# ittiam-systems/libxaac

Measured on AMD Instinct MI355X. Metric: decoded audio frames/s (1024-spl IMDCT + complex QMF + HQ SBR + parametric stereo, HE-AACv2), higher is better.
Workload: dtype int32

## Files before the change

libxaac_amd/csrc/sbr_core.h:

```cpp
#ifndef XAAC_SBR_CORE_H
#define XAAC_SBR_CORE_H

#include "fx.h"
#include "../../include/xaac_sbr.h"

#ifndef XS_TABLES_DECLARED
#define XS_TABLES_DECLARED
#if defined(__HIPCC__)
#define XAAC_TAB_QUAL static __device__ const
#include "tables_sbr.inc"
#undef XAAC_TAB_QUAL
#else
#include "tables_sbr.inc"
#endif
#endif

#define XS_MAXF XAAC_SBR_MAX_FREQ_COEFFS

FX_HD int32_t xs_shl(int32_t v, int s) { return (int32_t)((uint32_t)v << (s & 31)); }
FX_HD int32_t xs_sar(int32_t v, int s) { return v >> (s & 31); }
FX_HD int xs_pnorm32(int32_t a) { return fx_norm32(a); }
FX_HD int16_t xs_mult16_shl_sat(int16_t a, int16_t b) { return fx_sat16(((int32_t)a * b) >> 15); }
FX_HD int16_t xs_mult16_shl(int16_t a, int16_t b) { return (int16_t)(((int32_t)a * b) >> 15); }
FX_HD int16_t xs_mult16(int16_t a, int16_t b) { return (int16_t)(((int32_t)a * b) >> 16); }
// ... 1815 lines not shown
    st->harm_index = (int16_t)((harm0 + n) & 3);
  }
  cx.sync();
}


FX_HD uint64_t xs_alias_groups_pk(const XsCx &cx, const XsPass &ps, const XsLv &deg1p, const XsLv &alias_red, int nsb,
                                  XsLv &end) {
  XsLv f;
  f.fill(0);
  XS_LANES(l, 0, 64) {
    const int q = l / XS_PK, k = l & (XS_PK - 1);
    if (q < ps.n && k < nsb) f.own(l) = xs_alias_run_bits(k, nsb, deg1p.own(l), alias_red.own(l));
  }
  const uint64_t in_run = xs_ballot(cx, f, 1, 64), red = xs_ballot(cx, f, 2, 64);
  XsLv st;
  st.fill(0);
  XS_LANES(l, 0, 64) st.own(l) = xs_alias_group_at(in_run, red, l, l & ~(XS_PK - 1), nsb, end.own(l)) ? 1 : 0;
  return xs_ballot(cx, st, 1, 64);
}
FX_HD void xs_alias_reduction_pk(const XsCx &cx, const XsPass &ps, XsEnv &v, const XsLv &degp, const XsLv &deg1p, XsWork *w,
                                 uint64_t starts, const XsLv &end, int nsb) {
  if (starts == 0) return;
  XS_LANES(l, 0, 64) {
    w->fold_a[l][0] = v.est.own(l);
    w->fold_a[l][1] = v.gain.own(l);
  }
  cx.sync();
  XS_LANES(s, 0, 64) {
    if (!((starts >> s) & 1)) continue;
    int16_t amp_m, amp_e, gg_m, gg_e;
    xs_avggain(w->fold_a, s, end.own(s), &amp_m, &amp_e, &gg_m, &gg_e, 1);
    w->res_a[s][0] = amp_m;
    w->res_a[s][1] = amp_e;
    w->res_a[s][2] = gg_m;
    w->res_a[s][3] = gg_e;
    w->res_b[s][0] = (int16_t)end.own(s);
  }
  cx.sync();
  XsLv mine;
  mine.fill(-1);
  XS_LANES(l, 0, 64) {
    const int q = l / XS_PK, k = l & (XS_PK - 1);
    if (!(q < ps.n && k < nsb)) continue;
    const uint64_t below = starts & xs_mask_upto(l);
    if (!below) continue;
    const int s = 63 - xs_clz64(below);
    if (l >= w->res_b[s][0]) continue;
    mine.own(l) = s;
    xs_alias_mix_band((int16_t)degp.own(l), (int16_t)deg1p.own(l), k < nsb - 1, w->res_a[s][2], w->res_a[s][3],
                      v.est.own(l), v.gain.own(l), w->fold_b[l]);
  }
  cx.sync();
  XS_LANES(s, 0, 64) {
    if (!((starts >> s) & 1)) continue;
    xs_alias_compensation(w->fold_b, s, end.own(s), w->res_a[s][0], w->res_a[s][1], w->res_b[s][1], w->res_a[s][3]);
  }
  cx.sync();
  XS_LANES(l, 0, 64) {
    const int s = mine.own(l);
    if (s < 0) continue;
    v.gain.own(l) = xs_alias_compensate_band(v.gain.own(l), w->res_b[s][1], w->res_a[s][3]);
  }
  cx.sync();
}
FX_HD bool xs_pack_frame_ok(const XsCx &cx, const xaac_sbr_header *h) {
  const int nhi = cx.uni(h->num_sf_bands[1]), nlo = cx.uni(h->num_sf_bands[0]), nlf = cx.uni(h->num_lf_bands);
  const int sb_start = cx.uni(h->sub_band_start), sb_end = cx.uni(h->sub_band_end), nsb = sb_end - sb_start;
  if (!cx.uni(h->interpol_freq) || nhi < 1 || nlo < 1 || nsb < 1 || nsb > XS_PK) return false;
  if (cx.uni(h->freq_band_tbl_hi[0]) != sb_start || cx.uni(h->freq_band_tbl_lo[0]) != sb_start) return false;
  if (cx.uni(h->freq_band_tbl_hi[nhi]) != sb_end || cx.uni(h->freq_band_tbl_lo[nlo]) != sb_end) return false;
  int32_t bad = 0;
  XS_LANES(c, 0, nlf + 1) bad |= h->freq_band_tbl_lim[c] > nsb;
  return cx.wave_or(bad) == 0;
}

struct XsApplyHq {
  int32_t sl_even, sl_odd;
  int ls, rs, keep, col, step, kk, harm_lane;
  int16_t sg, snz;
  bool tone, noise, fi, live;
  int32_t hr, hr_keep;
};
template <int N, class Q>
FX_HD void xs_apply_slots_hq(const Q &x, XsApplyHq &a, int l, int &ph, int &harm) {
  int32_t rp[N], xr[N], xi[N];
  XS_UNROLL
  for (int j = 0; j < N; j++) rp[j] = XS_TAB_RAND(((ph + j * a.step) & 511) + 1 + a.kk);
  XS_UNROLL
  for (int j = 0; j < N; j++) {
    xr[j] = x(l + j, a.col);
    xi[j] = x.im(l + j, a.col);
  }
  XS_UNROLL
  for (int j = 0; j < N; j++) {
    int32_t re = fx_mul32x16(xr[j], a.sg), im = fx_mul32x16(xi[j], a.sg);
    re = (fx_shlw(re, a.ls) >> a.rs) & a.keep;
    im = (fx_shlw(im, a.ls) >> a.rs) & a.keep;
    const int hi = (a.harm_lane + j) & 3;
    const bool plus = a.fi != (hi == 1);
    const int32_t re_a = fx_add_sat(re, a.sl_even), re_s = fx_sub_sat(re, a.sl_even);
    const int32_t im_a = fx_add_sat(im, a.sl_odd), im_s = fx_sub_sat(im, a.sl_odd);
    const int32_t re_t = hi == 0 ? re_a : (hi == 2 ? re_s : re);
    const int32_t im_t = (hi & 1) ? (plus ? im_a : im_s) : im;
    const int32_t re_n = xs_mac16x16_shl_sat(re, (int16_t)(rp[j] >> 16), a.snz);
    const int32_t im_n = xs_mac16x16_shl_sat(im, (int16_t)rp[j], a.snz);
    xr[j] = a.tone ? re_t : (a.noise ? re_n : re);
    xi[j] = a.tone ? im_t : (a.noise ? im_n : im);
    a.hr |= (fx_abs_nrm(xr[j]) | fx_abs_nrm(xi[j])) & a.hr_keep;
  }
  if (a.live) {
    XS_UNROLL
    for (int j = 0; j < N; j++) {
      x(l + j, a.col) = xr[j];
      x.im(l + j, a.col) = xi[j];
    }
  }
  ph = (ph + N * a.step) & 511;
  harm = (harm + N) & 3;
  a.harm_lane = (a.harm_lane + N) & 3;
}

struct XsAdjMem {
  XsLv fb, fn;
  XsLv hr;
  int start_up, ph_index, harm_index, filt_buf_noise_e;
  bool two;
};
template <class ST>
FX_HD void xs_adj_load(const XsCx &cx, const ST *st, int nsb, XsAdjMem &m) {
  m.two = nsb <= 32;
  m.fb.fill(0);
  m.fn.fill(0);
  m.hr.fill(0);
  XS_LANES(li, 0, 64) {
    const int i = m.two ? li & 31 : li;
    if (i < nsb && i < XS_MAXF) {
      m.fb.own(li) = xs_me(st->filt_buf_me[2 * i], st->filt_buf_me[2 * i + 1]);
      m.fn.own(li) = st->filt_buf_noise_m[i];
    }
  }
  m.start_up = cx.uni(st->start_up);
  m.ph_index = cx.uni(st->ph_index);
  m.harm_index = cx.uni(st->harm_index);
  m.filt_buf_noise_e = cx.uni(st->filt_buf_noise_e);
}
template <class ST>
FX_HD void xs_adj_store(const XsCx &cx, ST *st, int nsb, const XsAdjMem &m) {
  XS_LANES(li, 0, m.two ? 32 : 64) {
    if (li < nsb && li < XS_MAXF) {
      st->filt_buf_me[2 * li] = xs_m(m.fb.own(li));
      st->filt_buf_me[2 * li + 1] = xs_e(m.fb.own(li));
      st->filt_buf_noise_m[li] = (int16_t)m.fn.own(li);
    }
  }
  XS_ONE {
    st->start_up = (int16_t)m.start_up;
    st->ph_index = (int16_t)m.ph_index;
    st->harm_index = (int16_t)m.harm_index;
    st->filt_buf_noise_e = (int16_t)m.filt_buf_noise_e;
  }
  cx.sync();
}

template <class Q>
FX_HD void xs_adapt_noise_gain_hq(const XsCx &cx, XsAdjMem &m, const XsEnv &v, int lane_off, int noise_e, int nsb, int skip,
                                  int s0, int s1, int input_e, int adj_e, int final_e, int sb_start, int noise_absc,
                                  int smooth_length, const Q &x) {
  const int bands = nsb - skip;
  const int start_up = m.start_up;
  const int ph0 = m.ph_index, harm0 = m.harm_index;
  const int fb_noise_e0 = start_up ? noise_e : m.filt_buf_noise_e;
  const bool two = m.two;
  XsLv gain_i, noise_i, sine_i;
  {
    XsLv idx;
    idx.fill(0);
    XS_LANES(li, 0, 64) idx.own(li) = ((two ? li & 31 : li) - skip + lane_off) & 63;
    gain_i = v.gain.gather(idx);
    noise_i = v.noise.gather(idx);
    sine_i = v.sine.gather(idx);
  }
  XS_LANES(li, 0, 64) {
    const int i = two ? li & 31 : li;
    const bool band = i >= skip && i < nsb;
    gain_i.own(li) = band ? gain_i.own(li) : 0;
    noise_i.own(li) = band ? noise_i.own(li) : 0;
    sine_i.own(li) = band ? sine_i.own(li) : 0;
    if (band) {
      int16_t g[2] = {xs_m(gain_i.own(li)), xs_e(gain_i.own(li))};
      if (start_up) {
        m.fb.own(li) = gain_i.own(li);
        m.fn.own(li) = xs_m(noise_i.own(li));
      } else {
        int16_t fb[2] = {xs_m(m.fb.own(li)), xs_e(m.fb.own(li))};
        xs_equalize_filt_buf(fb, g);
        m.fb.own(li) = xs_me(fb[0], fb[1]);
        gain_i.own(li) = xs_me(g[0], g[1]);
      }
    }
  }
  XS_T(29);
  XS_T(21);
  XS_LANES(li, 0, two ? 64 : nsb) {
    const int g = two ? li >> 5 : 0, i = two ? li & 31 : li;
    if (i >= nsb) continue;
    const int k = i - skip;
    const int16_t gm = xs_m(gain_i.own(li)), ge = xs_e(gain_i.own(li));
    const int16_t sm = xs_m(sine_i.own(li)), se = xs_e(sine_i.own(li));
    int16_t nl = xs_m(noise_i.own(li));
    int16_t fbm = xs_m(m.fb.own(li)), fbn = (int16_t)m.fn.own(li);
    int ne = noise_e, fbe = fb_noise_e0, ph = ph0, harm = harm0;
    int32_t hr = 0;
    int harm_lane0 = harm0;
    XS_KEEP(harm_lane0);
    const int col = sb_start + (k >= 0 ? k : 0), kk = k >= 0 ? k : 0;
    int l = s0;
    int n_smooth = s1 - s0 < smooth_length ? s1 - s0 : smooth_length;
    for (; n_smooth > 0; n_smooth--, l++) {
      int scale_change;
      if (l < Q::NS) {
        scale_change = adj_e - input_e;
      } else {
        scale_change = final_e - input_e;
        if (l == Q::NS && s0 < Q::NS) {
          const int diff = final_e - ne;
          ne = final_e;
          if (k >= 0) nl = xs_noise_rescale(nl, diff);
        }
      }
      fbn = xs_noise_rescale(fbn, fbe - ne);
      fbe = ne;
      const int32_t rp = XS_TAB_RAND((ph & 511) + 1 + kk);
      const int hi = harm;
      ph = (ph + bands) & 511;
      harm = (harm + 1) & 3;
      if (k < 0) continue;
      const int16_t smooth = XS_TAB_SMOOTH(l - s0);
      int16_t sg = gm, snz = nl;
      if (smooth) {
        const int16_t direct = fx_sat16(0x7fff - (int32_t)smooth);
        const int16_t t = (int16_t)(xs_mult16(smooth, fbm) + xs_mult16(direct, gm));
        const int16_t t1 = (int16_t)(xs_mult16(smooth, fbn) + xs_mult16(direct, nl));
        fbm = (int16_t)(t << 1);
        fbn = (int16_t)(t1 << 1);
        sg = fbm;
        snz = fbn;
      }
      const int16_t sc = (int16_t)((int16_t)scale_change - 1);
      int32_t re = fx_mul32x16(x(l, col), sg), im = fx_mul32x16(x.im(l, col), sg);
      const int shift = (int16_t)(ge - sc);
      if (shift > 0) {
        re = fx_shl(re, shift);
        im = fx_shl(im, shift);
      } else {
        re = fx_shr(re, -shift);
        im = fx_shr(im, -shift);
      }
      if (sm != 0) {
        const int tmp = (int16_t)(se - (int16_t)(ne - 16));
        int32_t sine_level;
        if (!(hi & 1)) {
          sine_level = tmp > 0 ? fx_shl(sm, tmp) : fx_shr(sm, tmp);
          re = hi == 0 ? fx_add_sat(re, sine_level) : fx_sub_sat(re, sine_level);
        } else {
          sine_level = tmp > 0 ? fx_shl(sm, tmp) : fx_shr(sm, -tmp);
          int fi = sb_start & 1;
          if (hi == 1) fi = !fi;
          if (k & 1) fi = !fi;
          im = fi ? fx_add_sat(im, sine_level) : fx_sub_sat(im, sine_level);
        }
      } else if (!noise_absc) {
        re = xs_mac16x16_shl_sat(re, (int16_t)(rp >> 16), snz);
        im = xs_mac16x16_shl_sat(im, (int16_t)rp, snz);
      }
      hr |= (g == 0 && l < Q::NS) ? (fx_abs_nrm(re) | fx_abs_nrm(im)) : 0;
      if (g == 0) {
        x(l, col) = re;
        x.im(l, col) = im;
      }
    }
    XS_T(30);
    while (l < s1) {
      const int seg_end = (l < Q::NS && s1 > Q::NS) ? Q::NS : s1;
      int scale_change;
      if (l < Q::NS) {
        scale_change = adj_e - input_e;
      } else {
        scale_change = final_e - input_e;
        if (l == Q::NS && s0 < Q::NS) {
          const int diff = final_e - ne;
          ne = final_e;
          if (k >= 0) nl = xs_noise_rescale(nl, diff);
        }
      }
      fbn = xs_noise_rescale(fbn, fbe - ne);
      fbe = ne;
      XsApplyHq a;
      a.sg = gm;
      a.snz = nl;
      {
        const int shift = (int16_t)(ge - (int16_t)((int16_t)scale_change - 1));
        const int b = (shift > 0 ? shift : -shift) & 0xff;
        a.ls = shift > 0 && b <= 31 ? b : 0;
        a.rs = shift > 0 ? 0 : (b < 31 ? b : 31);
        a.keep = shift > 0 && b > 31 ? 0 : -1;
      }
      const int tmp = (int16_t)(se - (int16_t)(ne - 16));
      a.sl_even = tmp > 0 ? fx_shl(sm, tmp) : fx_shr(sm, tmp);
      a.sl_odd = tmp > 0 ? fx_shl(sm, tmp) : fx_shr(sm, -tmp);
      a.tone = k >= 0 && sm != 0;
      a.noise = k >= 0 && sm == 0 && !noise_absc;
      a.fi = ((sb_start ^ kk) & 1) != 0;
      a.live = k >= 0;
      a.col = col;
      a.step = bands;
      a.kk = kk;
      a.hr = 0;
      a.hr_keep = (k >= 0 && l < Q::NS) ? -1 : 0;
      const int count = seg_end - l, half = two ? (count + 1) >> 1 : count;
      int lg = g ? l + half : l, phg = g ? (ph + half * bands) & 511 : ph, harmg = g ? (harm + half) & 3 : harm;
      const int end_g = g ? seg_end : l + half;
      a.harm_lane = (harm_lane0 + (lg - s0)) & 3;
      for (; lg + 8 <= end_g; lg += 8) xs_apply_slots_hq<8>(x, a, lg, phg, harmg);
      if (lg + 4 <= end_g) {
        xs_apply_slots_hq<4>(x, a, lg, phg, harmg);
        lg += 4;
      }
      if (lg + 2 <= end_g) {
        xs_apply_slots_hq<2>(x, a, lg, phg, harmg);
        lg += 2;
      }
      if (lg < end_g) {
        xs_apply_slots_hq<1>(x, a, lg, phg, harmg);
        lg += 1;
      }
      hr |= a.hr;
      ph = (ph + count * bands) & 511;
      harm = (harm + count) & 3;
      l = seg_end;
    }
    m.fb.own(li) = xs_me(k >= 0 ? gm : fbm, xs_e(m.fb.own(li)));
    m.fn.own(li) = k >= 0 ? nl : fbn;
    m.hr.own(li) |= hr;
  }
  cx.sync();
  XS_T(22);
  {
    const int n = s1 > s0 ? s1 - s0 : 0;
    int ne = noise_e;
    if (s0 < Q::NS && s1 > Q::NS) ne = final_e;
    m.start_up = 0;
    m.filt_buf_noise_e = n > 0 ? ne : fb_noise_e0;
    m.ph_index = (int16_t)((ph0 + n * bands) & 511);
    m.harm_index = (int16_t)((harm0 + n) & 3);
  }
}

struct XsCovHq {
  int32_t phi_11, phi_22, phi_01, phi_02, phi_12, phi_01_im, phi_02_im, phi_12_im;
};
template <class Q>
FX_HD void xs_covariance_hq(const Q &x, int k, int n0, int n1, int slots, bool first, XsCovHq *c) {
  int32_t p01 = 0, p01i = 0, p02 = 0, p02i = 0, p11 = 0, p12 = 0, p12i = 0, p22 = 0;
  int32_t r2 = fx_shr(x(n0 - 2, k), 3), i2 = fx_shr(x.im(n0 - 2, k), 3);
  int32_t r1 = fx_shr(x(n0 - 1, k), 3), i1 = fx_shr(x.im(n0 - 1, k), 3);
  if (first) {
    p22 = fx_add(xs_mul_hi16(r2, r2), xs_mul_hi16(i2, i2));
    p12 = fx_add(xs_mul_hi16(r1, r2), xs_mul_hi16(i1, i2));
    p12i = fx_sub(xs_mul_hi16(i1, r2), xs_mul_hi16(r1, i2));
  }
  XS_UNROLL4
  for (int n = n0; n < n1; n++) {
    const int32_t r0 = fx_shr(x(n, k), 3), i0 = fx_shr(x.im(n, k), 3);
    const int32_t t01 = fx_add(xs_mul_hi16(r0, r1), xs_mul_hi16(i0, i1));
    const int32_t t01i = fx_sub(xs_mul_hi16(i0, r1), xs_mul_hi16(r0, i1));
    const int32_t e1 = fx_add(xs_mul_hi16(r1, r1), xs_mul_hi16(i1, i1));
    p01 = fx_add(p01, t01);
    p01i = fx_add(p01i, t01i);
    p02 = fx_add(p02, fx_add(xs_mul_hi16(r0, r2), xs_mul_hi16(i0, i2)));
    p02i = fx_add(p02i, fx_sub(xs_mul_hi16(i0, r2), xs_mul_hi16(r0, i2)));
    p11 = fx_add(p11, e1);
    if (n < slots - 1) {
      p12 = fx_add(p12, t01);
      p12i = fx_add(p12i, t01i);
      p22 = fx_add(p22, e1);
    }
    r2 = r1;
    i2 = i1;
    r1 = r0;
    i1 = i0;
  }
  c->phi_11 = p11;
  c->phi_22 = p22;
  c->phi_01 = p01;
  c->phi_02 = p02;
  c->phi_12 = p12;
  c->phi_01_im = p01i;
  c->phi_02_im = p02i;
  c->phi_12_im = p12i;
}

FX_HD void xs_lpc_coeffs_hq(const XsCovHq *s, int16_t *a) {
  int32_t mx = fx_abs_nrm(s->phi_01) | fx_abs_nrm(s->phi_02) | fx_abs_nrm(s->phi_12) | s->phi_11 | s->phi_22 |
               fx_abs_nrm(s->phi_01_im) | fx_abs_nrm(s->phi_02_im) | fx_abs_nrm(s->phi_12_im);
  const int q = xs_pnorm32(mx);
  const int32_t p11 = xs_shl(s->phi_11, q), p22 = xs_shl(s->phi_22, q), p01 = xs_shl(s->phi_01, q),
                p02 = xs_shl(s->phi_02, q), p12 = xs_shl(s->phi_12, q), p01i = xs_shl(s->phi_01_im, q),
                p02i = xs_shl(s->phi_02_im, q), p12i = xs_shl(s->phi_12_im, q);
  const int32_t d = fx_shlw(fx_sub_sat(fx_mul32(p11, p22), fx_add_sat(fx_mul32(p12, p12), fx_mul32(p12i, p12i))), 1);
  int reset = 0;
  int16_t a1r = 0, a1i = 0, a0r = 0, a0i = 0;
  if (d != 0) {
    const int norm_d = fx_norm32(d);
    const int16_t inv_d = (int16_t)xs_fix_div(0x40000000, xs_shl(d, norm_d));
    const int32_t mod_d = fx_abs_sat(d);
    const int32_t tr = fx_sub_sat(fx_sub_sat(fx_mul32(p01, p12), fx_mul32(p01i, p12i)), fx_mul32(p02, p11)) >> 1;
    const int32_t ti = fx_sub_sat(fx_add_sat(fx_mul32(p01i, p12), fx_mul32(p01, p12i)), fx_mul32(p02i, p11)) >> 1;
    if (fx_abs_sat(tr) >= mod_d)
      reset = 1;
    else
      a1r = (int16_t)(xs_shl(fx_mul32x16(tr, inv_d), norm_d + 1) >> 15);
    if (fx_abs_sat(ti) >= mod_d)
      reset = 1;
    else
      a1i = (int16_t)(xs_shl(fx_mul32x16(ti, inv_d), norm_d + 1) >> 15);
  }
  if (p11 != 0) {
    const int norm = fx_norm32(p11);
    const int16_t inv = (int16_t)xs_fix_div(0x40000000, xs_shl(p11, norm));
    int32_t tr = fx_add_sat(fx_add(p01 >> 3, fx_mul32x16(p12, a1r)), fx_mul32x16(p12i, a1i));
    int32_t ti = fx_sub_sat(fx_add(p01i >> 3, fx_mul32x16(p12, a1i)), fx_mul32x16(p12i, a1r));
    tr = fx_shlw(tr, 1);
    ti = fx_shlw(ti, 1);
    if (fx_abs_sat(tr) >= p11)
      reset = 1;
    else
      a0r = (int16_t)(xs_shl(fx_mul32x16(fx_sub_sat(0, tr), inv), norm + 1) >> 15);
    if (fx_abs_sat(ti) >= p11)
      reset = 1;
    else
      a0i = (int16_t)(xs_shl(fx_mul32x16(fx_sub_sat(0, ti), inv), norm + 1) >> 15);
  }
  if (fx_add_sat((int32_t)a0r * a0r, (int32_t)a0i * a0i) >= 0x40000000) reset = 1;
  if (fx_add_sat((int32_t)a1r * a1r, (int32_t)a1i * a1i) >= 0x40000000) reset = 1;
  if (reset) a0r = a0i = a1r = a1i = 0;
  a[0] = a0r;
  a[1] = a0i;
  a[2] = a1r;
  a[3] = a1i;
}

template <class Q>
FX_HD void xs_patch_band_hq(const xaac_sbr_header *h, const Q &x, int lb, int hb, const int16_t *alpha,
                            const int32_t *bw_array, int start_idx, int stop_idx) {
  constexpr int kBwCap = XAAC_SBR_MAX_PATCHES - 1 < XAAC_SBR_MAX_NOISE_VALUES ? XAAC_SBR_MAX_PATCHES - 1 : XAAC_SBR_MAX_NOISE_VALUES;
  int bord[kBwCap];
  XS_UNROLL
  for (int i = 0; i < kBwCap; i++) bord[i] = h->bw_borders[i];
  int bi = 0;
  bool on = true;
  XS_UNROLL
  for (int i = 0; i < kBwCap; i++) {
    on = on && hb >= bord[i];
    bi += on ? 1 : 0;
  }
  int16_t bw = (int16_t)(bw_array[bi] >> 16);
  const int16_t a0r = xs_mult16_shl_sat(bw, alpha[0]), a0i = xs_mult16_shl_sat(bw, alpha[1]);
  bw = xs_mult16_shl_sat(bw, bw);
  const int16_t a1r = xs_mult16_shl_sat(bw, alpha[2]), a1i = xs_mult16_shl_sat(bw, alpha[3]);
  const int n = stop_idx - start_idx;
  const bool filt = bw > 0;
  const int16_t c0r = filt ? a0r : (int16_t)0, c0i = filt ? a0i : (int16_t)0, c1r = filt ? a1r : (int16_t)0,
                c1i = filt ? a1i : (int16_t)0;
  int32_t p2r = x(start_idx - 2, lb), p2i = x.im(start_idx - 2, lb);
  int32_t p1r = x(start_idx - 1, lb), p1i = x.im(start_idx - 1, lb);
  XS_UNROLL4
  for (int i = 0; i < n; i++) {
    const int32_t cr = x(start_idx + i, lb), ci = x.im(start_idx + i, lb);
    int32_t acc = fx_sub(fx_add(fx_sub(fx_mul32x16(p1r, c0r), fx_mul32x16(p1i, c0i)), fx_mul32x16(p2r, c1r)),
                         fx_mul32x16(p2i, c1i));
    x(start_idx + i, hb) = fx_add(cr >> 2, fx_shlw(acc, 1));
    acc = fx_add(fx_add_sat(fx_add_sat(fx_mul32x16(p1r, c0i), fx_mul32x16(p1i, c0r)), fx_mul32x16(p2r, c1i)),
                 fx_mul32x16(p2i, c1r));
    x.im(start_idx + i, hb) = fx_add(ci >> 2, fx_shlw(acc, 1));
    p2r = p1r;
    p2i = p1i;
    p1r = cr;
    p1i = ci;
  }
}

template <class ST, class Q>
FX_HD void xs_hf_generator_hq(const XsCx &cx, const xaac_sbr_header *h, ST *st, const Q &x, XsWork *w,
                              int start_idx, int last_slot_offset, int max_qmf_subband, const int32_t *invf_mode,
                              const int32_t *invf_mode_prev) {
  const int num_patches = cx.uni(h->num_patches);
  const int stop_idx = cx.uni(h->num_columns) + last_slot_offset;
  XS_PAR(i, 0, XAAC_SBR_MAX_PATCHES) w->bw_array[i] = 0;
  cx.sync();
  xs_invfilt_level_emphasis(cx, st->bw_array_prev, h->num_if_bands, invf_mode, invf_mode_prev, w->bw_array);
  const int actual_stop = cx.uni(
      (int16_t)(h->patch[num_patches - 1].dst_start_band + h->patch[num_patches - 1].num_bands_in_patch));
  {
    const int nz = actual_stop < Q::NB ? Q::NB - actual_stop : 0;
    XS_PAR(c, 0, 2 * nz) {
      const int col = c < nz ? actual_stop + c : Q::IM + actual_stop + (c - nz);
      XS_UNROLL4
      for (int l = start_idx; l < stop_idx; l++) x(l, col) = 0;
    }
  }
  const int start_patch = cx.uni(h->start_patch), stop_patch = cx.uni(h->stop_patch);
  XS_PAR(k, start_patch, stop_patch) {
    x(-2, k) = st->lpc_real[0][k];
    x(-1, k) = st->lpc_real[1][k];
    x.im(-2, k) = st->lpc_imag[0][k];
    x.im(-1, k) = st->lpc_imag[1][k];
  }
  cx.sync();
  XS_T(12);
  XsLv al01, al23, src;
  al01.fill(0);
  al23.fill(0);
  const int ncov = Q::LD ? cx.uni(h->num_columns) : Q::NS + 6;
  const int cw = stop_patch <= 16 ? 16 : (stop_patch <= 32 ? 32 : 64), cper = (ncov * cw + 63) / 64;
  XsLv cv[8];
  for (int i = 0; i < 8; i++) cv[i].fill(0);
  XS_LANES(c, 0, 64) {
    const int lb = c & (cw - 1), g = c / cw;
    const int n0 = g * cper, n1 = n0 + cper < ncov ? n0 + cper : ncov;
    if (lb >= start_patch && lb < stop_patch && n0 < n1) {
      XsCovHq part;
      xs_covariance_hq(x, lb, n0, n1, ncov, g == 0, &part);
      cv[0].own(c) = part.phi_11;
      cv[1].own(c) = part.phi_22;
      cv[2].own(c) = part.phi_01;
      cv[3].own(c) = part.phi_02;
      cv[4].own(c) = part.phi_12;
      cv[5].own(c) = part.phi_01_im;
      cv[6].own(c) = part.phi_02_im;
      cv[7].own(c) = part.phi_12_im;
    }
  }
  if (cw < 64)
    for (int i = 0; i < 8; i++) cv[i] = cv[i].fold(cw);
  XS_T(31);
  XS_LANES(lb, start_patch, stop_patch) {
    XsCovHq c;
    c.phi_11 = cv[0].own(lb);
    c.phi_22 = cv[1].own(lb);
    c.phi_01 = cv[2].own(lb);
    c.phi_02 = cv[3].own(lb);
    c.phi_12 = cv[4].own(lb);
    c.phi_01_im = cv[5].own(lb);
    c.phi_02_im = cv[6].own(lb);
    c.phi_12_im = cv[7].own(lb);
    int16_t alpha[4];
    xs_lpc_coeffs_hq(&c, alpha);
    al01.own(lb) = xs_me(alpha[0], alpha[1]);
    al23.own(lb) = xs_me(alpha[2], alpha[3]);
  }
  XS_T(13);
  XS_LANES(hb, 0, 64) {
    int best = -1;
    for (int patch = 0; patch < num_patches; patch++) {
      const xaac_sbr_patch *pp = &h->patch[patch];
      const int lb = hb - pp->dst_end_band;
      if (lb < pp->src_start_band || lb >= pp->src_end_band || lb < start_patch || lb >= stop_patch) continue;
      if (hb < max_qmf_subband) continue;
      if (lb >= best) best = lb;
    }
    src.own(hb) = best;
  }
  int32_t wide = 0;
  XS_LANES(hb, 0, 64) wide |= src.own(hb) >= 0 && (hb < max_qmf_subband || hb >= max_qmf_subband + 32);
  if (cx.wave_or(wide) == 0 && max_qmf_subband >= 0 && stop_idx - start_idx >= 8) {
    XsLv idx;
    idx.fill(0);
    XS_LANES(l, 0, 64) idx.own(l) = (max_qmf_subband + (l & 31)) & 63;
    const XsLv src2 = src.gather(idx);
    XsLv srcc;
    srcc.fill(0);
    XS_LANES(l, 0, 64) srcc.own(l) = (max_qmf_subband + (l & 31) < 64) ? src2.own(l) : -1;
    const XsLv b01 = al01.gather(srcc), b23 = al23.gather(srcc);
    const int mid = start_idx + ((stop_idx - start_idx + 1) >> 1);
    XS_LANES(l, 0, 64) {
      const int lb = srcc.own(l), hb = max_qmf_subband + (l & 31);
      if (lb >= 0) {
        const int16_t alpha[4] = {xs_m(b01.own(l)), xs_e(b01.own(l)), xs_m(b23.own(l)), xs_e(b23.own(l))};
        xs_patch_band_hq(h, x, lb, hb, alpha, w->bw_array, l < 32 ? start_idx : mid, l < 32 ? mid : stop_idx);
      }
    }
  } else {
    const XsLv a01 = al01.gather(src), a23 = al23.gather(src);
    XS_LANES(hb, 0, 64) {
      const int lb = src.own(hb);
      if (lb >= 0) {
        const int16_t alpha[4] = {xs_m(a01.own(hb)), xs_e(a01.own(hb)), xs_m(a23.own(hb)), xs_e(a23.own(hb))};
        xs_patch_band_hq(h, x, lb, hb, alpha, w->bw_array, start_idx, stop_idx);
      }
    }
  }
  cx.sync();
  XS_T(14);
  XS_PAR(i, 0, h->num_if_bands) st->bw_array_prev[i] = w->bw_array[i];
  cx.sync();
}

struct XsPendingAdjust {
  int b0, b1, first_start, sh_ov, sh_main;
};
template <class ST, class Q>
FX_HD int xs_calc_sbrenvelope(const XsCx &cx, const xaac_sbr_header *h, const xaac_sbr_frame *f,
                              const int16_t *env_sf_all, const int16_t *noise_floor_all, ST *st, const Q &x,
                              XsWork *w, const int16_t *rand_hi, const XsLv &deg64, XsPendingAdjust *pend = nullptr,
                              const int32_t *sf_words = nullptr) {
  const int num_env = cx.uni(f->num_env);
  const int16_t *border = f->border_vec;
  const int16_t *noise_floor = noise_floor_all;
  const int sb_start = cx.uni(h->sub_band_start), sb_end = cx.uni(h->sub_band_end);
  const int max_sb = cx.uni(f->max_qmf_subband_aac);
  const int nsb = sb_end - sb_start;
  const int skip = max_sb - sb_start;
  const int transient_env = cx.uni(f->transient_env);
  XsEnv v;
  v.est.fill(0);
  v.e_orig.fill(0);
  v.gain.fill(0);
  v.noise.fill(0);
  v.sine.fill(0);
  v.meta.fill(0);
  v.alias_red.fill(0);
  v.deg = deg64.shifted(cx, sb_start);
  v.deg1 = deg64.shifted(cx, sb_start + 1);
  xs_map_sineflags(cx, h->freq_band_tbl_hi, cx.uni(h->num_sf_bands[1]), f->add_harmonics, st, transient_env,
                   v.sine_mapped);
  int adj_e;
  {
    const int prev_sb = cx.uni(st->prev_max_qmf_subband_aac);
// ... 461 lines not shown
```

libxaac_amd/csrc/sbr_core_kernel.hip:

```cpp
#include <hip/hip_runtime.h>
#include <stddef.h>
#include <stdint.h>
#include <stdlib.h>

#ifdef XS_PROFILE
__shared__ long long xs_prof_last[4];
__shared__ unsigned xs_prof_acc[4][32];
#define XS_T(i)                                                  \
  do {                                                           \
    if ((threadIdx.x & 63) == 0) {                               \
      long long t_ = clock64();                                  \
      xs_prof_acc[threadIdx.x >> 6][i] += (unsigned)(t_ - xs_prof_last[threadIdx.x >> 6]); \
      xs_prof_last[threadIdx.x >> 6] = t_;                       \
    }                                                            \
  } while (0)
#endif
__shared__ int16_t xs_lds_inv_table[256];
__shared__ int16_t xs_lds_sqrt_table[258];
__shared__ int32_t xs_lds_rand_ph[568];
__shared__ int16_t xs_lds_rand_hi[568];
__shared__ int16_t xs_lds_small16[8 + 4 + 50];
__shared__ int32_t xs_lds_new_bw[16];
#define XS_TAB_LIMG(i) xs_lds_small16[i]
#define XS_TAB_SMOOTH(i) xs_lds_small16[8 + (i)]
// ... 130 lines not shown
    if (lane < NNF) s.noise_floor[lane] = r_nf;
    int32_t *m = reinterpret_cast<int32_t *>(&s.st);
    if (lane < 2) m[lane] = r_hd;
#pragma unroll
    for (int j = 0; j < NT; j++)
      if (lane + 64 * j < kTailWords) m[2 + lane + 64 * j] = r_t[j];
    for (int i = lane; i < 2 * ROW; i += 64) s.x[i] = 0;
    if (NS < 32)
      for (int i = lane; i < (32 - NS) * ROW; i += 64) s.x[(8 + NS) * ROW + i] = 0;
    if (!HQ)
      for (int i = lane; i < 128; i += 64) s.x[XAAC_SBR_X_ROWS * ROW + i] = 0;
  }
  const bool held = NB == 64 || lane < NB;
#pragma unroll
  for (int j = 0; j < NOV; j++) above |= held ? 0 : r_ov[j];
  auto store_matrix = [&]() {
    if (held) {
#pragma unroll
      for (int j = 0; j < NOV; j++) {
        const int row = HQ ? j >> 1 : j, part = HQ ? j & 1 : 0;
        s.x[(2 + row) * ROW + part * NB + lane] = r_ov[j];
      }
    }
#pragma unroll
    for (int j = 0; j < NAS; j++) {
      const int i = lane + 64 * j;
      const int row = HQ ? (i >> 6) : (i >> 5), col = HQ ? ((i & 31) + ((i & 32) ? Q::IM : 0)) : (i & 31);
      s.x[(8 + row) * ROW + col] = r_an[j];
    }
    for (int i = lane; i < NS * (HQ ? 2 : 1) * (NB - 32); i += 64) {
      const int row = i / ((HQ ? 2 : 1) * (NB - 32)), c = i % ((HQ ? 2 : 1) * (NB - 32));
      s.x[(8 + row) * ROW + (c < NB - 32 ? 32 + c : Q::IM + 32 + (c - (NB - 32)))] = 0;
    }
  };
  xs_wave_sync();
#ifdef XS_PROFILE
  XS_T(24);
#endif

  const XsCx cx = {lane, 64};
  const Q x = {s.x};
  if (lane == 0) s.st.lb_scale = 0;
  const int refused = xs_side_info_bad(cx, &s.h, f, &s.st, 0, NS);
  if (NB < 64) {
    int32_t top = 0;
    if (!refused) {
      const int32_t lim[4] = {s.st.syn_usb, s.st.syn_lsb, s.st.codec_usb, s.st.prev_max_qmf_subband_aac};
      for (int i = 0; i < 4; i++) top = lim[i] > top ? lim[i] : top;
      if (f->apply_processing) {
        top = s.h.sub_band_end > top ? s.h.sub_band_end : top;
        top = f->max_qmf_subband_aac > top ? f->max_qmf_subband_aac : top;
        if (lane <= s.h.num_sf_bands[1] && s.h.freq_band_tbl_hi[lane] > top) top = s.h.freq_band_tbl_hi[lane];
        if (lane <= s.h.num_sf_bands[0] && s.h.freq_band_tbl_lo[lane] > top) top = s.h.freq_band_tbl_lo[lane];
        if (lane < s.h.num_patches) {
          const xaac_sbr_patch *pp = &s.h.patch[lane];
          const int a = pp->src_end_band + pp->dst_end_band, b = pp->dst_start_band + pp->num_bands_in_patch;
          top = a > top ? a : top;
          top = b > top ? b : top;
        }
      }
    }
    if (cx.wave_max(top) > NB || cx.wave_or(above) != 0) return false;
  }
  const int apply = __builtin_amdgcn_readfirstlane((int)f->apply_processing);
  const int old_lsb = __builtin_amdgcn_readfirstlane((int)s.st.prev_max_qmf_subband_aac);
  const int new_lsb = __builtin_amdgcn_readfirstlane((int)f->max_qmf_subband_aac);
  const bool in_regs = !refused && !(apply && new_lsb != old_lsb && old_lsb > 0);
  if (!in_regs) store_matrix();
  if (apply && !refused) xs_rescale_x_overlap(cx, &s.h, f, &s.st, x);
  xs_wave_sync();
  if (lane == 0) {
    s.st.st_lb_scale = 0;
    s.st.lb_scale = HQ ? -8 : -10;
  }
  xs_wave_sync();
  int save_lb_scale = 0;
  XsPendingAdjust pend = {0, 0, 0, 0, 0};
  XS_T(26);
#ifdef XS_SKIP_CORE
  const int rc = 0;
  if (in_regs) store_matrix();
#else
  int rc = -1;
  if (in_regs) {
    const int usb = __builtin_amdgcn_readfirstlane((int)s.st.codec_usb);
    int32_t m_ov = 1, m_an = 1;
    const bool low_ov = lane < usb, low_an = (lane & 31) < usb;
#pragma unroll
    for (int j = 0; j < NOV; j++) m_ov |= low_ov ? fx_abs_nrm(r_ov[j]) : 0;
#pragma unroll
    for (int j = 0; j < NAS; j++) m_an |= low_an ? fx_abs_nrm(r_an[j]) : 0;
    const int reserve = xs_pnorm32(cx.wave_or(m_an)), reserve_ov1 = xs_pnorm32(cx.wave_or(m_ov));
    const XsBfp b = xs_bfp_shifts<HQ>(cx, &s.st, usb, reserve, reserve_ov1);
    if (b.sh_ov != 0) {
#pragma unroll
      for (int j = 0; j < NOV; j++) r_ov[j] = low_ov ? xs_adjust_word(r_ov[j], b.sh_ov) : r_ov[j];
    }
    if (b.sh_main != 0) {
#pragma unroll
      for (int j = 0; j < NAS; j++) r_an[j] = low_an ? xs_adjust_word(r_an[j], b.sh_main) : r_an[j];
    }
    store_matrix();
    save_lb_scale = b.save_lb_scale;
    xs_wave_sync();
    XS_T(1);
    rc = xs_sbr_core_tail(cx, &s.h, f, p.frame[ch].int_env_sf_arr, reinterpret_cast<const int16_t *>(s.noise_floor), &s.st, x,
                          &s.w, HQ ? nullptr : xs_lds_rand_hi, b, &pend, r_sf);
  } else if (!refused) {
    rc = xs_sbr_core(cx, &s.h, f, p.frame[ch].int_env_sf_arr, reinterpret_cast<const int16_t *>(s.noise_floor), &s.st, x, &s.w,
                     HQ ? nullptr : xs_lds_rand_hi, &save_lb_scale);
  }
#endif
  xs_wave_sync();
#ifdef XS_PROFILE
  XS_T(15);
#endif

  if (lane == 0) {
    int16_t *par = p.syn_par + 8 * (size_t)ch;
    par[0] = s.st.lb_scale;
    par[1] = s.st.ov_lb_scale;
    par[2] = s.st.hb_scale;
    par[3] = s.st.st_syn_scale;
    par[4] = s.st.syn_lsb;
    par[5] = s.st.syn_usb;
    par[6] = 0;
    par[7] = 0;
    s.st.ov_lb_scale = (int16_t)save_lb_scale;
#ifndef XS_PROFILE
    if (p.status) p.status[ch] = rc;
#endif
  }
  xs_wave_sync();
  {
    constexpr int NW = (NS + 6) * ROWG / 64;
    const bool held = NB == 64 || lane < NB;
    const int lane_h = held ? lane : 0;
    const bool adj_band = lane >= pend.b0 && lane < pend.b1;
    const auto counts = [](int sh, int &l, int &r) {
      sh = sh > 31 ? 31 : (sh < -31 ? -31 : sh);
      l = sh > 0 ? sh : 0;
      r = sh < 0 ? -sh : 0;
    };
    int ov_l, ov_r, mn_l, mn_r;
    counts(pend.sh_ov, ov_l, ov_r);
    counts(pend.sh_main, mn_l, mn_r);
#pragma unroll
    for (int j0 = 0; j0 < NW; j0 += 8) {
      int32_t t[8];
#pragma unroll
      for (int j = 0; j < 8; j++)
        if (j0 + j < NW) {
          const int row = HQ ? (j0 + j) >> 1 : j0 + j, part = HQ ? (j0 + j) & 1 : 0;
          int32_t v = s.x[(2 + row) * ROW + part * NB + lane_h];
          if (row < NS) {
            const int sl = row < pend.first_start ? ov_l : mn_l, sr = row < pend.first_start ? ov_r : mn_r;
            const int32_t w = (int32_t)((uint32_t)v << sl) >> sr;
            v = adj_band ? w : v;
          }
          t[j] = held ? v : 0;
        }
#pragma unroll
      for (int j = 0; j < 8; j++)
        if (j0 + j < NW) gx[2 * ROWG + 64 * (j0 + j) + lane] = t[j];
    }
  }
  {
    int32_t *gw = reinterpret_cast<int32_t *>(gst);
#pragma unroll
    for (int j = 0; j < 6; j++) {
      const int row = HQ ? j >> 1 : j, part = HQ ? j & 1 : 0;
      const bool held = NB == 64 || lane < NB;
      int32_t v = s.x[(2 + NS + row) * ROW + part * NB + (held ? lane : 0)];
      if (NS + row < pend.first_start && lane >= pend.b0 && lane < pend.b1) {
        const int sh = pend.sh_ov > 31 ? 31 : (pend.sh_ov < -31 ? -31 : pend.sh_ov);
        v = sh > 0 ? (int32_t)((uint32_t)v << sh) : (v >> -sh);
      }
      gw[offsetof(xaac_sbr_state, overlap) / 4 + 64 * j + lane] = held ? v : 0;
    }
    const int32_t *m = reinterpret_cast<const int32_t *>(&s.st);
    if (lane < 2) gw[kHeadOff / 4 + lane] = m[lane];
    copy_words(gw + kTailOff / 4, m + 2, kTailWords, lane);
  }
#ifdef XS_PROFILE
  XS_T(25);
  xs_wave_sync();
  if (lane < 32 && p.status) atomicAdd(reinterpret_cast<unsigned long long *>(p.status) + lane, (unsigned long long)xs_prof_acc[threadIdx.x >> 6][lane]);
#endif
  return true;
}

template <int HQ, int THREADS>
__device__ __forceinline__ void stage_tables(int tid) {
// ... 159 lines not shown
```

Baseline: 17.28 million.

## Specialise HQ envelope apply by tone/noise mode, derive cross covariances from sums

The per-slot HQ gain application is templated on tone, noise and headroom flags and dispatched through a wave-uniform mode, so random-phase table loads, noise MACs and tone arithmetic are skipped when a frame has no sinusoids or noise. The covariance pass now accumulates only five terms and reconstructs phi_12 and phi_22 from phi_01 and phi_11 by correcting the end samples, which removes the conditional accumulation inside the loop. The fallback path that does not hold the matrix in registers now does its own headroom and adjust steps and then calls the shared tail routine instead of the separate full core. The eight-way template instantiation adds code size, and the end-correction relies on saturating adds matching the original sums.

Measured after the change: 17.31 million (median of 5 runs). No clear change (+0.2%).

```diff
diff --git a/libxaac_amd/csrc/sbr_core.h b/libxaac_amd/csrc/sbr_core.h
--- a/libxaac_amd/csrc/sbr_core.h
+++ b/libxaac_amd/csrc/sbr_core.h
@@ -1921,11 +1921,13 @@
   bool tone, noise, fi, live;
   int32_t hr, hr_keep;
 };
-template <int N, class Q>
+template <int N, bool TONE, bool NOISE, bool HR, class Q>
 FX_HD void xs_apply_slots_hq(const Q &x, XsApplyHq &a, int l, int &ph, int &harm) {
   int32_t rp[N], xr[N], xi[N];
-  XS_UNROLL
-  for (int j = 0; j < N; j++) rp[j] = XS_TAB_RAND(((ph + j * a.step) & 511) + 1 + a.kk);
+  if (NOISE) {
+    XS_UNROLL
+    for (int j = 0; j < N; j++) rp[j] = XS_TAB_RAND(((ph + j * a.step) & 511) + 1 + a.kk);
+  }
   XS_UNROLL
   for (int j = 0; j < N; j++) {
     xr[j] = x(l + j, a.col);
@@ -1936,17 +1938,25 @@
     int32_t re = fx_mul32x16(xr[j], a.sg), im = fx_mul32x16(xi[j], a.sg);
     re = (fx_shlw(re, a.ls) >> a.rs) & a.keep;
     im = (fx_shlw(im, a.ls) >> a.rs) & a.keep;
-    const int hi = (a.harm_lane + j) & 3;
-    const bool plus = a.fi != (hi == 1);
-    const int32_t re_a = fx_add_sat(re, a.sl_even), re_s = fx_sub_sat(re, a.sl_even);
-    const int32_t im_a = fx_add_sat(im, a.sl_odd), im_s = fx_sub_sat(im, a.sl_odd);
-    const int32_t re_t = hi == 0 ? re_a : (hi == 2 ? re_s : re);
-    const int32_t im_t = (hi & 1) ? (plus ? im_a : im_s) : im;
-    const int32_t re_n = xs_mac16x16_shl_sat(re, (int16_t)(rp[j] >> 16), a.snz);
-    const int32_t im_n = xs_mac16x16_shl_sat(im, (int16_t)rp[j], a.snz);
-    xr[j] = a.tone ? re_t : (a.noise ? re_n : re);
-    xi[j] = a.tone ? im_t : (a.noise ? im_n : im);
-    a.hr |= (fx_abs_nrm(xr[j]) | fx_abs_nrm(xi[j])) & a.hr_keep;
+    int32_t re_n = re, im_n = im;
+    if (NOISE) {
+      re_n = xs_mac16x16_shl_sat(re, (int16_t)(rp[j] >> 16), a.snz);
+      im_n = xs_mac16x16_shl_sat(im, (int16_t)rp[j], a.snz);
+    }
+    if (TONE) {
+      const int hi = (a.harm_lane + j) & 3;
+      const bool plus = a.fi != (hi == 1);
+      const int32_t re_a = fx_add_sat(re, a.sl_even), re_s = fx_sub_sat(re, a.sl_even);
+      const int32_t im_a = fx_add_sat(im, a.sl_odd), im_s = fx_sub_sat(im, a.sl_odd);
+      const int32_t re_t = hi == 0 ? re_a : (hi == 2 ? re_s : re);
+      const int32_t im_t = (hi & 1) ? (plus ? im_a : im_s) : im;
+      xr[j] = a.tone ? re_t : (NOISE && a.noise ? re_n : re);
+      xi[j] = a.tone ? im_t : (NOISE && a.noise ? im_n : im);
+    } else {
+      xr[j] = re_n;
+      xi[j] = im_n;
+    }
+    if (HR) a.hr |= fx_abs_nrm(xr[j]) | fx_abs_nrm(xi[j]);
   }
   if (a.live) {
     XS_UNROLL
@@ -1957,7 +1967,33 @@
   }
   ph = (ph + N * a.step) & 511;
   harm = (harm + N) & 3;
-  a.harm_lane = (a.harm_lane + N) & 3;
+  if (TONE) a.harm_lane = (a.harm_lane + N) & 3;
+}
+template <bool TONE, bool NOISE, bool HR, class Q>
+FX_HD void xs_apply_segment_hq(const Q &x, XsApplyHq &a, int lg, int end_g, int ph, int harm) {
+  for (; lg + 8 <= end_g; lg += 8) xs_apply_slots_hq<8, TONE, NOISE, HR>(x, a, lg, ph, harm);
+  if (lg + 4 <= end_g) {
+    xs_apply_slots_hq<4, TONE, NOISE, HR>(x, a, lg, ph, harm);
+    lg += 4;
+  }
+  if (lg + 2 <= end_g) {
+    xs_apply_slots_hq<2, TONE, NOISE, HR>(x, a, lg, ph, harm);
+    lg += 2;
+  }
+  if (lg < end_g) xs_apply_slots_hq<1, TONE, NOISE, HR>(x, a, lg, ph, harm);
+}
+template <class Q>
+FX_HD void xs_apply_segment_hq(int mode, const Q &x, XsApplyHq &a, int lg, int end_g, int ph, int harm) {
+  switch (mode & 7) {
+    case 0: xs_apply_segment_hq<false, false, false>(x, a, lg, end_g, ph, harm); break;
+    case 1: xs_apply_segment_hq<false, false, true>(x, a, lg, end_g, ph, harm); break;
+    case 2: xs_apply_segment_hq<false, true, false>(x, a, lg, end_g, ph, harm); break;
+    case 3: xs_apply_segment_hq<false, true, true>(x, a, lg, end_g, ph, harm); break;
+    case 4: xs_apply_segment_hq<true, false, false>(x, a, lg, end_g, ph, harm); break;
+    case 5: xs_apply_segment_hq<true, false, true>(x, a, lg, end_g, ph, harm); break;
+    case 6: xs_apply_segment_hq<true, true, false>(x, a, lg, end_g, ph, harm); break;
+    default: xs_apply_segment_hq<true, true, true>(x, a, lg, end_g, ph, harm); break;
+  }
 }
 
 struct XsAdjMem {
@@ -2039,6 +2075,13 @@
       }
     }
   }
+  int32_t tone_any = 0;
+  XS_LANES(li, 0, 64) tone_any |= xs_m(sine_i.own(li)) != 0 ? 4 : 0;
+#ifdef XS_WALK_WHOLE_BODY
+  const int walk_mode = 7;
+#else
+  const int walk_mode = Q::LD ? 7 : cx.wave_or(tone_any) | (noise_absc ? 0 : 2);
+#endif
   XS_T(29);
   XS_T(21);
   XS_LANES(li, 0, two ? 64 : nsb) {
@@ -2161,20 +2204,8 @@
       int lg = g ? l + half : l, phg = g ? (ph + half * bands) & 511 : ph, harmg = g ? (harm + half) & 3 : harm;
       const int end_g = g ? seg_end : l + half;
       a.harm_lane = (harm_lane0 + (lg - s0)) & 3;
-      for (; lg + 8 <= end_g; lg += 8) xs_apply_slots_hq<8>(x, a, lg, phg, harmg);
-      if (lg + 4 <= end_g) {
-        xs_apply_slots_hq<4>(x, a, lg, phg, harmg);
-        lg += 4;
-      }
-      if (lg + 2 <= end_g) {
-        xs_apply_slots_hq<2>(x, a, lg, phg, harmg);
-        lg += 2;
-      }
-      if (lg < end_g) {
-        xs_apply_slots_hq<1>(x, a, lg, phg, harmg);
-        lg += 1;
-      }
-      hr |= a.hr;
+      xs_apply_segment_hq(cx.uni(walk_mode | (l < Q::NS ? 1 : 0)), x, a, lg, end_g, phg, harmg);
+      hr |= a.hr & a.hr_keep;
       ph = (ph + count * bands) & 511;
       harm = (harm + count) & 3;
       l = seg_end;
@@ -2200,44 +2231,61 @@
   int32_t phi_11, phi_22, phi_01, phi_02, phi_12, phi_01_im, phi_02_im, phi_12_im;
 };
 template <class Q>
-FX_HD void xs_covariance_hq(const Q &x, int k, int n0, int n1, int slots, bool first, XsCovHq *c) {
-  int32_t p01 = 0, p01i = 0, p02 = 0, p02i = 0, p11 = 0, p12 = 0, p12i = 0, p22 = 0;
+FX_HD void xs_covariance_hq(const Q &x, int k, int n0, int n1, XsCovHq *c) {
+  int32_t p01 = 0, p01i = 0, p02 = 0, p02i = 0, p11 = 0;
   int32_t r2 = fx_shr(x(n0 - 2, k), 3), i2 = fx_shr(x.im(n0 - 2, k), 3);
   int32_t r1 = fx_shr(x(n0 - 1, k), 3), i1 = fx_shr(x.im(n0 - 1, k), 3);
-  if (first) {
-    p22 = fx_add(xs_mul_hi16(r2, r2), xs_mul_hi16(i2, i2));
-    p12 = fx_add(xs_mul_hi16(r1, r2), xs_mul_hi16(i1, i2));
-    p12i = fx_sub(xs_mul_hi16(i1, r2), xs_mul_hi16(r1, i2));
-  }
   XS_UNROLL4
   for (int n = n0; n < n1; n++) {
     const int32_t r0 = fx_shr(x(n, k), 3), i0 = fx_shr(x.im(n, k), 3);
-    const int32_t t01 = fx_add(xs_mul_hi16(r0, r1), xs_mul_hi16(i0, i1));
-    const int32_t t01i = fx_sub(xs_mul_hi16(i0, r1), xs_mul_hi16(r0, i1));
-    const int32_t e1 = fx_add(xs_mul_hi16(r1, r1), xs_mul_hi16(i1, i1));
-    p01 = fx_add(p01, t01);
-    p01i = fx_add(p01i, t01i);
+    p01 = fx_add(p01, fx_add(xs_mul_hi16(r0, r1), xs_mul_hi16(i0, i1)));
+    p01i = fx_add(p01i, fx_sub(xs_mul_hi16(i0, r1), xs_mul_hi16(r0, i1)));
     p02 = fx_add(p02, fx_add(xs_mul_hi16(r0, r2), xs_mul_hi16(i0, i2)));
     p02i = fx_add(p02i, fx_sub(xs_mul_hi16(i0, r2), xs_mul_hi16(r0, i2)));
-    p11 = fx_add(p11, e1);
-    if (n < slots - 1) {
-      p12 = fx_add(p12, t01);
-      p12i = fx_add(p12i, t01i);
-      p22 = fx_add(p22, e1);
-    }
+    p11 = fx_add(p11, fx_add(xs_mul_hi16(r1, r1), xs_mul_hi16(i1, i1)));
     r2 = r1;
     i2 = i1;
     r1 = r0;
     i1 = i0;
   }
   c->phi_11 = p11;
-  c->phi_22 = p22;
   c->phi_01 = p01;
   c->phi_02 = p02;
-  c->phi_12 = p12;
   c->phi_01_im = p01i;
   c->phi_02_im = p02i;
-  c->phi_12_im = p12i;
+}
+template <class Q>
+FX_HD void xs_covariance_hq_ends(const Q &x, int k, int slots, XsCovHq *c) {
+  const int32_t ar = fx_shr(x(-2, k), 3), ai = fx_shr(x.im(-2, k), 3), br = fx_shr(x(-1, k), 3), bi = fx_shr(x.im(-1, k), 3);
+  const int32_t yr = fx_shr(x(slots - 2, k), 3), yi = fx_shr(x.im(slots - 2, k), 3);
+  const int32_t zr = fx_shr(x(slots - 1, k), 3), zi = fx_shr(x.im(slots - 1, k), 3);
+  c->phi_12 = fx_add(fx_sub(c->phi_01, fx_add(xs_mul_hi16(zr, yr), xs_mul_hi16(zi, yi))),
+                     fx_add(xs_mul_hi16(br, ar), xs_mul_hi16(bi, ai)));
+  c->phi_12_im = fx_add(fx_sub(c->phi_01_im, fx_sub(xs_mul_hi16(zi, yr), xs_mul_hi16(zr, yi))),
+                        fx_sub(xs_mul_hi16(bi, ar), xs_mul_hi16(br, ai)));
+  c->phi_22 = fx_add(fx_sub(c->phi_11, fx_add(xs_mul_hi16(yr, yr), xs_mul_hi16(yi, yi))),
+                     fx_add(xs_mul_hi16(ar, ar), xs_mul_hi16(ai, ai)));
+}
+
+template <class Q>
+FX_HD void xs_covariances_hq(const XsCx &cx, const Q &x, int start_patch, int stop_patch, int slots, XsLv *cv) {
+  const int cw = stop_patch <= 16 ? 16 : (stop_patch <= 32 ? 32 : 64), cper = (slots * cw + 63) / 64;
+  for (int i = 0; i < 5; i++) cv[i].fill(0);
+  XS_LANES(c, 0, 64) {
+    const int lb = c & (cw - 1), g = c / cw;
+    const int n0 = g * cper, n1 = n0 + cper < slots ? n0 + cper : slots;
+    if (lb >= start_patch && lb < stop_patch && n0 < n1) {
+      XsCovHq part;
+      xs_covariance_hq(x, lb, n0, n1, &part);
+      cv[0].own(c) = part.phi_11;
+      cv[1].own(c) = part.phi_01;
+      cv[2].own(c) = part.phi_02;
+      cv[3].own(c) = part.phi_01_im;
+      cv[4].own(c) = part.phi_02_im;
+    }
+  }
+  if (cw < 64)
+    for (int i = 0; i < 5; i++) cv[i] = cv[i].fold(cw);
 }
 
 FX_HD void xs_lpc_coeffs_hq(const XsCovHq *s, int16_t *a) {
@@ -2362,38 +2410,17 @@
   al01.fill(0);
   al23.fill(0);
   const int ncov = Q::LD ? cx.uni(h->num_columns) : Q::NS + 6;
-  const int cw = stop_patch <= 16 ? 16 : (stop_patch <= 32 ? 32 : 64), cper = (ncov * cw + 63) / 64;
-  XsLv cv[8];
-  for (int i = 0; i < 8; i++) cv[i].fill(0);
-  XS_LANES(c, 0, 64) {
-    const int lb = c & (cw - 1), g = c / cw;
-    const int n0 = g * cper, n1 = n0 + cper < ncov ? n0 + cper : ncov;
-    if (lb >= start_patch && lb < stop_patch && n0 < n1) {
-      XsCovHq part;
-      xs_covariance_hq(x, lb, n0, n1, ncov, g == 0, &part);
-      cv[0].own(c) = part.phi_11;
-      cv[1].own(c) = part.phi_22;
-      cv[2].own(c) = part.phi_01;
-      cv[3].own(c) = part.phi_02;
-      cv[4].own(c) = part.phi_12;
-      cv[5].own(c) = part.phi_01_im;
-      cv[6].own(c) = part.phi_02_im;
-      cv[7].own(c) = part.phi_12_im;
-    }
-  }
-  if (cw < 64)
-    for (int i = 0; i < 8; i++) cv[i] = cv[i].fold(cw);
+  XsLv cv[5];
+  xs_covariances_hq(cx, x, start_patch, stop_patch, ncov, cv);
   XS_T(31);
   XS_LANES(lb, start_patch, stop_patch) {
     XsCovHq c;
     c.phi_11 = cv[0].own(lb);
-    c.phi_22 = cv[1].own(lb);
-    c.phi_01 = cv[2].own(lb);
-    c.phi_02 = cv[3].own(lb);
-    c.phi_12 = cv[4].own(lb);
-    c.phi_01_im = cv[5].own(lb);
-    c.phi_02_im = cv[6].own(lb);
-    c.phi_12_im = cv[7].own(lb);
+    c.phi_01 = cv[1].own(lb);
+    c.phi_02 = cv[2].own(lb);
+    c.phi_01_im = cv[3].own(lb);
+    c.phi_02_im = cv[4].own(lb);
+    xs_covariance_hq_ends(x, lb, ncov, &c);
     int16_t alpha[4];
     xs_lpc_coeffs_hq(&c, alpha);
     al01.own(lb) = xs_me(alpha[0], alpha[1]);
diff --git a/libxaac_amd/csrc/sbr_core_kernel.hip b/libxaac_amd/csrc/sbr_core_kernel.hip
--- a/libxaac_amd/csrc/sbr_core_kernel.hip
+++ b/libxaac_amd/csrc/sbr_core_kernel.hip
@@ -236,6 +236,7 @@
   if (in_regs) store_matrix();
 #else
   int rc = -1;
+  XsBfp b = {0, 0, 0, 0};
   if (in_regs) {
     const int usb = __builtin_amdgcn_readfirstlane((int)s.st.codec_usb);
     int32_t m_ov = 1, m_an = 1;
@@ -245,7 +246,7 @@
 #pragma unroll
     for (int j = 0; j < NAS; j++) m_an |= low_an ? fx_abs_nrm(r_an[j]) : 0;
     const int reserve = xs_pnorm32(cx.wave_or(m_an)), reserve_ov1 = xs_pnorm32(cx.wave_or(m_ov));
-    const XsBfp b = xs_bfp_shifts<HQ>(cx, &s.st, usb, reserve, reserve_ov1);
+    b = xs_bfp_shifts<HQ>(cx, &s.st, usb, reserve, reserve_ov1);
     if (b.sh_ov != 0) {
 #pragma unroll
       for (int j = 0; j < NOV; j++) r_ov[j] = low_ov ? xs_adjust_word(r_ov[j], b.sh_ov) : r_ov[j];
@@ -255,14 +256,20 @@
       for (int j = 0; j < NAS; j++) r_an[j] = low_an ? xs_adjust_word(r_an[j], b.sh_main) : r_an[j];
     }
     store_matrix();
+  } else if (!refused) {
+    const int usb = __builtin_amdgcn_readfirstlane((int)s.st.codec_usb);
+    const int reserve = xs_headroom(cx, x, 0, usb, 6, 6 + NS), reserve_ov1 = xs_headroom(cx, x, 0, usb, 0, 6);
+    b = xs_bfp_shifts<HQ>(cx, &s.st, usb, reserve, reserve_ov1);
+    xs_adjust(cx, x, 0, usb, 0, 6, b.sh_ov);
+    xs_adjust(cx, x, 0, usb, 6, 6 + NS, b.sh_main);
+    xs_clear(cx, x, 32, NB, 6, 6 + NS);
+  }
+  if (!refused) {
     save_lb_scale = b.save_lb_scale;
     xs_wave_sync();
     XS_T(1);
     rc = xs_sbr_core_tail(cx, &s.h, f, p.frame[ch].int_env_sf_arr, reinterpret_cast<const int16_t *>(s.noise_floor), &s.st, x,
                           &s.w, HQ ? nullptr : xs_lds_rand_hi, b, &pend, r_sf);
-  } else if (!refused) {
-    rc = xs_sbr_core(cx, &s.h, f, p.frame[ch].int_env_sf_arr, reinterpret_cast<const int16_t *>(s.noise_floor), &s.st, x, &s.w,
-                     HQ ? nullptr : xs_lds_rand_hi, &save_lb_scale);
   }
 #endif
   xs_wave_sync();
```
